# RemoteSensingTools/vSmartMOM.jl

Hardware: AMD Instinct MI355X
Metric: spectral-points/s (whole node) for rt_run, O2-A band (higher is better)
Workload: dtype f64; 1 GPU; C2: O2-A 759-770 nm, nStokes=3, Nquad=20 (N=60), 40 layers, 10000 spectral points/GPU, m=0..2, Rayleigh+synthetic O2 absorption, Lambertian 0.15; ranks=1, collective_backend=none (1 rank), N=60, layers=40, points_per_gpu=10000, fourier_moments=3

## Files before the change

include/vsmartmom_hip.h:

```cpp
#ifndef VSMARTMOM_HIP_H
#define VSMARTMOM_HIP_H

#include <stddef.h>
#include <stdint.h>

#ifdef __cplusplus
extern "C" {
#endif

typedef enum vsm_status {
  VSM_OK = 0,
  VSM_ERR_INVALID_ARG = 1,
  VSM_ERR_UNSUPPORTED = 2,
  VSM_ERR_HIP = 3,
  VSM_ERR_NO_DEVICE = 4
} vsm_status;

typedef enum vsm_iface {
  VSM_IFACE_00 = 0,
  VSM_IFACE_01 = 1,
  VSM_IFACE_10 = 2,
  VSM_IFACE_11 = 3
} vsm_iface;

// ... 334 lines not shown
                       size_t workspace_bytes, vsm_run** run);
int vsm_run_create_ex_f64(const vsm_quad_f64* q, int S, int nm, const int* m_h, const int* coupling_h, void* workspace,
                          size_t workspace_bytes, unsigned flags, vsm_run** run);
int vsm_run_create_ex_f32(const vsm_quad_f32* q, int S, int nm, const int* m_h, const int* coupling_h, void* workspace,
                          size_t workspace_bytes, unsigned flags, vsm_run** run);
int vsm_run_create_view_f64(const vsm_quad_f64* q, int S, int nm, const int* m_h, const int* coupling_h, void* workspace,
                            size_t workspace_bytes, unsigned flags, int nrows, const int* rows_h, vsm_run** run);
int vsm_run_create_view_f32(const vsm_quad_f32* q, int S, int nm, const int* m_h, const int* coupling_h, void* workspace,
                            size_t workspace_bytes, unsigned flags, int nrows, const int* rows_h, vsm_run** run);
int vsm_run_create_view_f64(const vsm_quad_f64* q, int S, int nm, const int* m_h, const int* coupling_h, void* workspace,
                            size_t workspace_bytes, unsigned flags, int nrows, const int* rows_h, vsm_run** run);
int vsm_run_create_view_f32(const vsm_quad_f32* q, int S, int nm, const int* m_h, const int* coupling_h, void* workspace,
                            size_t workspace_bytes, unsigned flags, int nrows, const int* rows_h, vsm_run** run);
int vsm_run_layer_f64(vsm_run* run, int ndoubl, const double* dtau, const double* varpi, const double* tau_sum,
                      const double* F0, int ncomp, const double* const* Zpp, const double* const* Zmp, long long z_stride,
                      const double* fcomp, int toa, const int* layer_coupling_h, void* stream);
int vsm_run_layer_f32(vsm_run* run, int ndoubl, const float* dtau, const float* varpi, const float* tau_sum,
                      const float* F0, int ncomp, const float* const* Zpp, const float* const* Zmp, long long z_stride,
                      const float* fcomp, int toa, const int* layer_coupling_h, void* stream);
int vsm_run_export_f64(vsm_run* run, const vsm_composite_f64* comps, void* stream);
int vsm_run_export_f32(vsm_run* run, const vsm_composite_f32* comps, void* stream);
int vsm_run_import_f64(vsm_run* run, const vsm_composite_f64* comps, void* stream);
int vsm_run_import_f32(vsm_run* run, const vsm_composite_f32* comps, void* stream);
int vsm_run_zw_tail(vsm_run* run);
int vsm_run_view_rows(vsm_run* run, int nrows, const int* rows_h);
int vsm_run_view_block(const vsm_run* run, int block, int* im, int* n, int* nv, int* local_rows);
int vsm_run_view_rows(vsm_run* run, int nrows, const int* rows_h);
int vsm_run_view_block(const vsm_run* run, int block, int* im, int* n, int* nv, int* local_rows);
int vsm_run_destroy(vsm_run* run);
int vsm_stokes_coupling_f64(int N, int n_stokes, int nblocks, const double* Zpp, const double* Zmp, int* mask_d, void* stream);
int vsm_stokes_coupling_f32(int N, int n_stokes, int nblocks, const float* Zpp, const float* Zmp, int* mask_d, void* stream);

typedef struct vsm_added_rs_f64 {
  double *ier_mp, *iet_pp, *ier_pm, *iet_mm;
  double *ieJ0_p, *ieJ0_m;
  int K;
  int reserved;
} vsm_added_rs_f64;
typedef struct vsm_added_rs_f32 {
  float *ier_mp, *iet_pp, *ier_pm, *iet_mm;
  float *ieJ0_p, *ieJ0_m;
  int K;
  int reserved;
} vsm_added_rs_f32;
typedef struct vsm_composite_rs_f64 {
  double *ieR_mp, *ieR_pm, *ieT_pp, *ieT_mm;
// ... 149 lines not shown
```

vsmartmom.jl_amd/_lib.py:

```python
from __future__ import annotations

import ctypes as C
import os

_HERE = os.path.dirname(os.path.abspath(__file__))
LIB_PATH = os.environ.get("VSM_LIB_PATH") or os.path.join(_HERE, "lib", "libvsmartmom_hip.so")


class VSMError(RuntimeError):
    pass


class vsm_quad_f64(C.Structure):
    _fields_ = [("mu", C.c_void_p), ("wt", C.c_void_p), ("N", C.c_int), ("n_stokes", C.c_int),
                ("i_mu0", C.c_int), ("mu0", C.c_double)]


class vsm_quad_f32(C.Structure):
    _fields_ = [("mu", C.c_void_p), ("wt", C.c_void_p), ("N", C.c_int), ("n_stokes", C.c_int),
                ("i_mu0", C.c_int), ("mu0", C.c_float)]


class vsm_added(C.Structure):
    _fields_ = [("r_mp", C.c_void_p), ("t_pp", C.c_void_p), ("r_pm", C.c_void_p), ("t_mm", C.c_void_p),
# ... 101 lines not shown
    "vsm_lambertian_surface_lin_{T}": (_I, [_P, _I, _I, "{R}", _I, _P, _P, _I, _P, _P, _P, _P]),
    "vsm_postprocess_vza_lin_{T}": (_I, [_I, _I, _I, _I, _I, _P, _P, _P, _P, _P, _P, _P]),
    "vsm_doubling_inelastic_work_elems": (_SZ, [_I, _I, _I]),
    "vsm_interaction_inelastic_work_elems": (_SZ, [_I, _I, _I]),
    "vsm_elemental_inelastic_rrs_{T}": (_I, [_P, _I, _I, _I, _P, _P, _P, _P, _P, _P]),
    "vsm_doubling_inelastic_rrs_{T}": (_I, [_I, _I, _I, _I, _P, _P, _P, _P, _P, _P]),
    "vsm_interaction_inelastic_rrs_{T}": (_I, [_I, _I, _I, _P, _P, _P, _P, _P, _P, _P]),
    "vsm_copy_added_to_composite_ie_{T}": (_I, [_I, _I, _P, _P, _P]),
    "vsm_postprocess_vza_ie_{T}": (_I, [_I, _I, _I, _I, _I, _P, _P, _P, _P, _P, _P, _P]),
    "vsm_ss_column_{T}": (_I, [_P, _I, _I, _I, _P, _P, _P, _P, _P, _P, _P, _P, _P, _P, _I, _P, _P, _P, _P, _P, _P, _P]),
    "vsm_ss_column_lin_{T}": (_I, [_P, _I, _I, _I, _I, _I, _I, _I, _I, _P, _P, _P, _P, _P, _P, _P, _P, _P, _P, _I, _P, _P, _P, _P, _P, _P, _P,
                                   _P, _P, _I, _P, _P, _P, _P, _P]),
    "vsm_ss_column_rrs_{T}": (_I, [_P, _I, _I, _I, _I, _P, _P, _P, _P, _P, _P, _P, _P, _I, _I, _P, _P, _P, _P, _P]),
    "vsm_run_supported": (_I, [_I, _I, _I]),
    "vsm_run_workspace_bytes": (_SZ, [_I, _I, _I, _I, _P]),
    "vsm_run_supported_f32": (_I, [_I, _I, _I]),
    "vsm_run_workspace_bytes_f32": (_SZ, [_I, _I, _I, _I, _P]),
    "vsm_run_create_{T}": (_I, [_P, _I, _I, _P, _P, _P, _SZ, _P]),
    "vsm_run_create_ex_{T}": (_I, [_P, _I, _I, _P, _P, _P, _SZ, C.c_uint, _P]),
    "vsm_run_create_view_{T}": (_I, [_P, _I, _I, _P, _P, _P, _SZ, C.c_uint, _I, _P, _P]),
    "vsm_run_layer_{T}": (_I, [_P, _I, _P, _P, _P, _P, _I, _P, _P, _LL, _P, _I, _P, _P]),
    "vsm_run_export_{T}": (_I, [_P, _P, _P]),
    "vsm_run_import_{T}": (_I, [_P, _P, _P]),
    "vsm_run_zw_tail": (_I, [_P]),
    "vsm_run_view_rows": (_I, [_P, _I, _P]),
    "vsm_run_view_block": (_I, [_P, _I, _P, _P, _P, _P]),
    "vsm_run_destroy": (_I, [_P]),
    "vsm_stokes_coupling_{T}": (_I, [_I, _I, _I, _P, _P, _P, _P]),
    "vsm_level_radiance_work_elems": (_SZ, [_I, _I]),
    "vsm_level_radiance_{T}": (_I, [_I, _I, _I, _I, _P, _P, _P, _P, _P, _LL, _P, _P, _P, _P, _P, _P, _P]),
    "vsm_level_radiance_oplevel_{T}": (_I, [_I, _I, _I, _I, _P, _P, _P, _P, _P, _LL, _P, _P, _P, _P, _P, _P, _P]),
    "vsm_level_radiance_src_{T}": (_I, [_I, _I, _I, _I, _P, _P, _P, _I, _P, _P, _LL, _P, _P, _P, _P, _P, _P, _P]),
    "vsm_level_radiance_ie_{T}": (_I, [_I, _I, _I, _I, _P, _I, _P, _P, _P, _P, _LL, _P, _P, _P, _P, _P, _P, _P, _P, _P, _P, _P]),
    "vsm_level_radiance_lin_{T}": (_I, [_I, _I, _I, _I, _I, _I, _P, _P, _P, _P, _LL, _P, _P, _P, _LL, _P, _P, _LL, _LL, _P, _P, _P, _P, _P,
                                        _P]),
    "vsm_test_lds_mm_{T}": (_I, [_I, _I, _P, _P, _P, _P]),
    "vsm_test_lds_inv_{T}": (_I, [_I, _I, _P, _P, _I, _P, _P]),
    "vsm_test_poison_lds": (_I, [_P]),
}


def exported_symbols():
    out = []
    for name in _SIGS:
        if "{T}" in name:
            out += [name.format(T="f64"), name.format(T="f32")]
# ... 89 lines not shown
```

vsmartmom.jl_amd/core_rt.py:

```python
from __future__ import annotations

import ctypes as C
import dataclasses
import math
import os
from dataclasses import dataclass
from typing import List, Optional

import numpy as np
import torch

from . import _lib
from . import host_model as H
from .architectures import GPU, CPU, architecture, array_type, devi, synchronize_if_gpu, to_host

IFACE = {"00": 0, "01": 1, "10": 2, "11": 3}
MOMENT_BATCH = 4
MOMENT_BATCH_MAX = 24
MOMENT_BATCHING = True
THERMAL_FUSION = True
NATIVE_RUN = True
NATIVE_SOURCES_ONLY = True
NATIVE_VIEW_ROWS = True
VIEW_ROWS_MAX = 16
NATIVE_ZW_TAIL = True
NATIVE_DROPIN = True
REFERENCE_ORDER = False


def _require_gpu(arch):
    if not isinstance(arch, GPU):
        raise _lib.VSMError("vsmartmom.jl_amd provides the MI355X path only; architecture %r has no compute path here "
                            "(no CPU fallback by design)" % (arch,))
    if not torch.cuda.is_available():
        raise _lib.VSMError("no MI355X visible to HIP (torch.cuda.is_available() is False)")
    if arch.device_index != torch.cuda.current_device():
        raise _lib.VSMError("architecture GPU(%d) is not the current HIP device (%d): one process per GPU -- call "
                            "torch.cuda.set_device(%d) first" % (arch.device_index, torch.cuda.current_device(),
                                                                 arch.device_index))


def _torch_dtype(FT):
    return torch.float64 if np.dtype(FT) == np.float64 else torch.float32


def _stream_ptr():
    return C.c_void_p(torch.cuda.current_stream().cuda_stream)
# ... 76 lines not shown
class AddedLayer:

    def __init__(self, FT, arch, N, nSpec, shared=False, d_symmetric=0):
        dev, dt = devi(arch), _torch_dtype(FT)
        sm = 1 if shared else nSpec
        z = lambda: torch.zeros((sm, N, N), dtype=dt, device=dev)
        self.r_mp, self.t_pp = z(), z()
        self.d_symmetric = int(d_symmetric)
        self.r_pm, self.t_mm = (None, None) if self.d_symmetric else (z(), z())
        self.j0_p = torch.zeros((nSpec, N), dtype=dt, device=dev)
        self.j0_m = torch.zeros((nSpec, N), dtype=dt, device=dev)
        self.N, self.nSpec, self.shared, self.dtype = N, nSpec, shared, dt

    def cstruct(self):
        return _lib.vsm_added(self.r_mp.data_ptr(), self.t_pp.data_ptr(),
                              0 if self.r_pm is None else self.r_pm.data_ptr(),
                              0 if self.t_mm is None else self.t_mm.data_ptr(),
                              self.j0_p.data_ptr(), self.j0_m.data_ptr(), 0 if self.shared else self.N * self.N,
                              self.d_symmetric, 0)


def _composite_field(name):
    def fget(self):
        return self.materialize()._arr[name]

    def fset(self, value):
        self.materialize()._arr[name] = value
    return property(fget, fset)


class CompositeLayer:

    def __init__(self, FT, arch, N, nSpec):
        dev, dt = devi(arch), _torch_dtype(FT)
        z = lambda: torch.zeros((nSpec, N, N), dtype=dt, device=dev)
        self._native = None
        self._sources_only = False
        self._view_rows = None
        self._native_ws = None
        self._arr = dict(R_mp=z(), R_pm=z(), T_pp=z(), T_mm=z(), J0_p=torch.zeros((nSpec, N), dtype=dt, device=dev),
                         J0_m=torch.zeros((nSpec, N), dtype=dt, device=dev))
        self.N, self.nSpec, self.dtype = N, nSpec, dt

    R_mp, R_pm, T_pp = _composite_field("R_mp"), _composite_field("R_pm"), _composite_field("T_pp")
    T_mm, J0_p, J0_m = _composite_field("T_mm"), _composite_field("J0_p"), _composite_field("J0_m")

    def materialize(self):
        slot = self._native
        if slot is None:
            return self
        self._native = None
        try:
            cc = (_lib.vsm_composite * 1)(self._cstruct_raw())
            _lib.call("vsm_run_export", self.dtype, slot.run, cc, _stream_ptr())
        finally:
            _lib.lib().vsm_run_destroy(slot.run)
        return self

    def drop_native(self):
        slot, self._native = self._native, None
        if slot is not None:
            _lib.lib().vsm_run_destroy(slot.run)

    def _cstruct_raw(self):
        a = self._arr
        return _lib.vsm_composite(a["R_mp"].data_ptr(), a["R_pm"].data_ptr(), a["T_pp"].data_ptr(), a["T_mm"].data_ptr(),
                                  a["J0_p"].data_ptr(), a["J0_m"].data_ptr())

    def cstruct(self):
        self.materialize()
        return self._cstruct_raw()

    def __del__(self):
        try:
            self.drop_native()
        except Exception:
            pass


def make_added_layer(FT, arch, dims, nSpec, shared=False, d_symmetric=0) -> AddedLayer:
    _require_gpu(arch)
    return AddedLayer(FT, arch, dims[0], nSpec, shared, d_symmetric)


def make_composite_layer(FT, arch, dims, nSpec) -> CompositeLayer:
    _require_gpu(arch)
    return CompositeLayer(FT, arch, dims[0], nSpec)


@dataclass
class DeviceLayerOptics:
    tau: torch.Tensor
    varpi: torch.Tensor
    Zpp: torch.Tensor
# ... 77 lines not shown

_work_cache = {}


def layer_forward_multi_(tau_sum, dtau, F0, props_list, ms, ndoubl: int, dq: DeviceQuad, toa: bool, comps, added: AddedLayer):
    nm = len(ms)
    p0 = props_list[0]
    q, a = dq.cstruct(), added.cstruct()
    dtype = comps[0].dtype
    carr = (type(comps[0].cstruct()) * nm)(*[c.cstruct() for c in comps])
    marr = (C.c_int * nm)(*[int(m) for m in ms])
    zpp = (C.c_void_p * nm)(*[p.Zpp.data_ptr() for p in props_list])
    zmp = (C.c_void_p * nm)(*[p.Zmp.data_ptr() for p in props_list])
    ncomp = 0 if p0.fcomp is None else int(p0.fcomp.shape[1])
    _lib.call("vsm_layer_forward_multi", dtype, C.byref(q), comps[0].nSpec, nm, marr, ndoubl, _ptr(dtau), _ptr(p0.varpi),
              _ptr(tau_sum), _ptr(F0), ncomp, zpp, zmp, 0 if ncomp else p0.z_stride, _ptr(p0.fcomp), None, 1 if toa else 0,
              carr, C.byref(a), _stream_ptr())


def run_layer_native_(run, nm: int, ndoubl: int, dtau, varpi, tau_sum, F0, ncomp: int, zpp, zmp, z_stride: int, fcomp, toa: bool,
                      layer_coupling=None, dtype=torch.float64):
    _lib.call("vsm_run_layer", dtype, run, ndoubl, _ptr(dtau), _ptr(varpi), _ptr(tau_sum), _ptr(F0), ncomp, zpp, zmp, z_stride,
              _ptr(fcomp), 1 if toa else 0, layer_coupling, _stream_ptr())


def interaction_(scattering_interface: str, comp: CompositeLayer, added: AddedLayer, oplevel: bool = False,
                 work: Optional[torch.Tensor] = None):
    a, c = added.cstruct(), comp.cstruct()
    N, S = comp.N, comp.nSpec
    fused = (scattering_interface == "11" and not oplevel
             and N <= _lib.lib().vsm_fused_max_n(8 if comp.dtype == torch.float64 else 4))
    if not fused and work is None:
        key = (N, S, comp.dtype, str(comp.R_mp.device))
        work = _work_cache.get(key)
        if work is None:
            _work_cache.clear()
            work = _lib.poison(torch.empty(int(_lib.lib().vsm_interaction_work_elems(N, S)), dtype=comp.dtype, device=comp.R_mp.device))
            _work_cache[key] = work
    name = "vsm_interaction_oplevel" if oplevel else "vsm_interaction"
    _lib.call(name, comp.dtype, IFACE[scattering_interface], N, S, C.byref(c), C.byref(a), _ptr(work), _stream_ptr())


_phi_cache = {}


def brdf_azimuth_quadrature(arch, FT):
# ... 39 lines not shown
        _lib.call("vsm_lambertian_surface_spectral", added_surface.dtype, C.byref(q), added_surface.nSpec, m, _ptr(rho),
                  _ptr(tau_sum), C.byref(a), _stream_ptr())
        return
    if not added_surface.shared:
        raise _lib.VSMError("surface AddedLayer must be allocated with shared=True")
    if isinstance(surface, H.LambertianSurfaceScalar):
        surface = surface.albedo
    if isinstance(surface, (int, float)):
        alb = C.c_double(surface) if added_surface.dtype == torch.float64 else C.c_float(surface)
        _lib.call("vsm_lambertian_surface", added_surface.dtype, C.byref(q), added_surface.nSpec, m, alb, _ptr(tau_sum),
                  C.byref(a), _stream_ptr())
        return
    if isinstance(surface, BRDF_SURFACES):
        if rho is None:
            rho, _ = reflectance(surface, dq, m, arch, FT)
        _lib.call("vsm_brdf_surface", added_surface.dtype, C.byref(q), added_surface.nSpec, m, _ptr(rho), _ptr(tau_sum),
                  C.byref(a), _stream_ptr())
        return
    raise _lib.VSMError("surface %r is not built in this backend (LambertianSurfaceScalar / Legendre / Spline, CoxMunkSurface, "
                        "rpvSurfaceScalar, RossLiSurfaceScalar)"
                        % (surface,))


def apply_ss_correction_(R_SFI: torch.Tensor, surf: H.CoxMunkSurface, pol, vza, vaz, mu0, tau_total: torch.Tensor, m_max: int,
                         arch, FT):
    nV, S = len(vza), int(R_SFI.shape[0])
    ctype = C.c_double if R_SFI.dtype == torch.float64 else C.c_float
    mu_v = (ctype * nV)(*[float(FT(H.cosd(v))) for v in vza])
    dph = (ctype * nV)(*[float(FT(math.radians(float(a)))) for a in vaz])
    coef = torch.empty((pol.n, nV), dtype=R_SFI.dtype, device=R_SFI.device)
    phi, w = brdf_azimuth_quadrature(arch, FT)
    cs = _coxmunk_cstruct(surf, R_SFI.dtype)
    _lib.call("vsm_coxmunk_ss_correction", R_SFI.dtype, C.byref(cs), pol.n, S, nV, mu_v, dph, ctype(float(mu0)), int(m_max),
              int(phi.numel()), _ptr(phi), _ptr(w), _ptr(tau_total), _ptr(coef), _ptr(R_SFI), _stream_ptr())
    return coef


def postprocessing_vza_(pol: H.PolarizationType, comp: CompositeLayer, vza, vaz, qp: H.QuadPoints, m: int, weight: float,
                        R_SFI: torch.Tensor, T_SFI: torch.Tensor):
    n, nV = pol.n, len(vza)
    row0 = (C.c_int * nV)()
    ctype = C.c_double if comp.dtype == torch.float64 else C.c_float
    w = (ctype * (nV * n))()
    for v in range(nV):
        imu = int(np.argmin(np.abs(qp.qp_mu - qp.qp_mu.dtype.type(H.cosd(vza[v])))))
        row0[v] = imu * n
# ... 1 lines not shown
        ws = [c, c, s, s][:n]
        for k in range(n):
            w[v + nV * k] = weight * ws[k]
    _lib.call("vsm_postprocess_vza", comp.dtype, comp.N, n, comp.nSpec, nV, row0, w, _ptr(comp.J0_m), _ptr(comp.J0_p),
              _ptr(R_SFI), _ptr(T_SFI), _stream_ptr())


def _vza_rows_weights(pol, vza, vaz, qp, m, weight, dtype):
    n, nV = pol.n, len(vza)
    row0 = (C.c_int * nV)()
    ctype = C.c_double if dtype == torch.float64 else C.c_float
    w = (ctype * (nV * n))()
    for v in range(nV):
        imu = int(np.argmin(np.abs(qp.qp_mu - qp.qp_mu.dtype.type(H.cosd(vza[v])))))
        row0[v] = imu * n
        c, s = H.cosd(m * vaz[v]), H.sind(m * vaz[v])
        for k in range(n):
            w[v + nV * k] = weight * [c, c, s, s][k]
    return row0, w


def interaction_hdrf_(pol, comp: CompositeLayer, added_surface: AddedLayer, m: int, dq: DeviceQuad, vza, vaz, qp, weight: float,
                      hdr_J: torch.Tensor, hdr: torch.Tensor, bhr_uw: torch.Tensor, bhr_dw: torch.Tensor):
    q, c, a = dq.cstruct(), comp.cstruct(), added_surface.cstruct()
    _lib.call("vsm_interaction_hdrf", comp.dtype, C.byref(q), comp.nSpec, m, C.byref(c), C.byref(a), _ptr(hdr_J), _ptr(bhr_uw),
              _ptr(bhr_dw), _stream_ptr())
    row0, w = _vza_rows_weights(pol, vza, vaz, qp, m, weight, comp.dtype)
    _lib.call("vsm_postprocess_vza_hdrf", comp.dtype, comp.N, pol.n, comp.nSpec, len(vza), row0, w, _ptr(hdr_J), _ptr(hdr),
              _stream_ptr())


def init_layer(props: DeviceLayerOptics, qp: H.QuadPoints, FT, numerics: H.RTNumericalParameters, arch):
    dtau_h, nd = H.get_dtau_ndoubl(props.tau_h, props.varpi_h, qp, FT, numerics)
    return array_type(arch)(dtau_h), nd


@dataclass
class NativeSlot:
    run: C.c_void_p
    m: int
    coupling: int
    grp_of: List[int]


def stokes_groups(n_stokes: int, coupling: int) -> List[int]:
    adj = [[a == b or coupling < 0 or bool((coupling >> (4 * a + b)) & 1) or bool((coupling >> (4 * b + a)) & 1)
            for b in range(n_stokes)] for a in range(n_stokes)]
# ... 378 lines not shown
        if self.layers_only:
            raise _lib.VSMError("Scene(layers_only=True) holds no composite layer: it feeds rt_run_ss only")
        self.R_SFI.zero_()
        self.T_SFI.zero_()
        self.hdr.zero_()
        if self.S == 0:
            return self.R_SFI, self.T_SFI
        self.added.j0_p.zero_()
        eps2 = 2 * np.finfo(FT).eps
        has_noscat = any(ly["props"].max_tau_varpi <= eps2 for ly in self.moments[0]["layers"])
        sequential = trace is not None or not MOMENT_BATCHING or has_noscat or REFERENCE_ORDER
        want = max(MOMENT_BATCH, min(MOMENT_BATCH_MAX, 4096 // max(self.S, 1)))
        nb = 1 if sequential else min(want, len(self.moments))
        while len(self._composites) < nb:
            self._composites.append(make_composite_layer(FT, self.arch, (self.N, self.N), self.S))
        native = self._native_moments() if trace is None and not has_noscat and not REFERENCE_ORDER else set()
        walk_src = streams is None and trace is None and not has_noscat
        if getattr(self, "_view_rows", None) is None:
            self._view_rows = view_rows_of(pol, model.vza, self.qp)
        view_rows = self._view_rows if streams is None else None
        for c in self._composites:
            c._sources_only = walk_src and REFERENCE_ORDER
            c._view_rows = view_rows if c._sources_only else None
        for g0 in range(0, len(self.moments), nb):
            group = self.moments[g0:g0 + nb]
            comps = self._composites[:len(group)]
            nat = [k for k in range(len(group)) if (g0 + k) in native]
            if nat:
                self._run_layers_native([group[k] for k in nat], [comps[k] for k in nat], sources_only=streams is None,
                                        view_rows=view_rows)
            rest = [k for k in range(len(group)) if (g0 + k) not in native]
            group_l, comps_l = [group[k] for k in rest], [comps[k] for k in rest]
            for iz in range(self.Nz if rest else 0):
                ly0 = group_l[0]["layers"][iz]
                if len(group_l) > 1 and ly0["props"].max_tau_varpi > eps2 and (iz == 0 or ly0["iface"] == "11"):
                    layer_forward_multi_(ly0["tau_sum"], ly0["dtau"], self.F0, [mom["layers"][iz]["props"] for mom in group_l],
                                         [mom["m"] for mom in group_l], ly0["nd"], self.dq, iz == 0, comps_l, self.added)
                    continue
                for mom, comp in zip(group_l, comps_l):
                    ly = mom["layers"][iz]
                    rt_kernel_(pol, self.added, comp, ly["props"], ly["iface"], ly["tau_sum"], mom["m"], self.dq,
                               self.arch, iz + 1, self.F0, FT, model.numerics, dtau=ly["dtau"], ndoubl=ly["nd"], trace=trace,
                               work=self.work, keep_added=has_noscat)
            for mom, comp in zip(group, comps):
                m = mom["m"]
                weight = FT(0.5 / math.pi) if m == 0 else FT(1.0 / math.pi)
                create_surface_layer_(model.surface, self.added_surface, m, self.dq, mom["tau_sum_surface"], rho=mom["rho"])
                interaction_(mom["iface_surface"], comp, self.added_surface, work=self.work)
                if self.compute_hdrf:
                    interaction_hdrf_(pol, comp, self.added_surface, m, self.dq, model.vza, model.vaz, self.qp, float(weight),
                                      self.hdr_J, self.hdr, self.bhr_uw, self.bhr_dw)
                postprocessing_vza_(pol, comp, model.vza, model.vaz, self.qp, m, float(weight), self.R_SFI, self.T_SFI)
                thermal_pass = self.thermal_B is not None and (m == 0 or (m == 1 and self._thermal_carry))
                if thermal_pass:
                    self._thermal_slot(mom, float(weight))
                if streams is not None:
                    Jm, Jp = comp.J0_m.clone(), comp.J0_p.clone()
                    if thermal_pass:
                        Jm += self._th_comp.J0_m
                        Jp += self._th_comp.J0_p
                    streams.append(dict(m=m, weight=float(weight), R_mp=comp.R_mp.clone(), T_pp=comp.T_pp.clone(), J0_m=Jm, J0_p=Jp))
        for c in self._composites:
            c._sources_only = False
            c._view_rows = None
        if isinstance(model.surface, H.CoxMunkSurface) and self.ss_correction:
            apply_ss_correction_(self.R_SFI, model.surface, pol, model.vza, model.vaz, self.qp.mu0,
                                 self.moments[-1]["tau_sum_surface"], model.m_max, self.arch, FT)
        return self.R_SFI, self.T_SFI

    def _native_moments(self):
        if not NATIVE_RUN or getattr(self, "coupling", None) is None or not self.moments:
            return set()
        eps2 = 2 * np.finfo(self.FT).eps
        for iz, ly in enumerate(self.moments[0]["layers"]):
            p = ly["props"]
            if p.max_tau_varpi <= eps2 or (iz > 0 and ly["iface"] != "11") or (p.fcomp is not None and p.fcomp.shape[1] > 4):
                return set()
        return {i for i, mom in enumerate(self.moments) if run_supported(self.dt, self.N, self.pol.n, int(self.coupling[mom["m"]]))}

    def _run_layers_native(self, group, comps, sources_only: bool = True, export_at=None, view_rows=None):
        L = _lib.lib()
        nm, N, S, ns = len(group), self.N, self.S, self.pol.n
        marr = (C.c_int * nm)(*[int(mom["m"]) for mom in group])
        carr = (C.c_int * nm)(*[int(self.coupling[mom["m"]]) for mom in group])
        nbytes = run_workspace_bytes(self.dt, N, ns, S, nm, carr)
        ws = getattr(self, "_native_ws", None)
        if ws is None or ws.numel() * 8 < nbytes:
            ws = self._native_ws = _lib.poison(torch.empty(max(nbytes // 8, 2), dtype=torch.float64, device=self.dev))
        q = self.dq.cstruct()
        run = C.c_void_p()
        run_create_(self.dt, q, S, nm, marr, carr, ws, nbytes, sources_only, view_rows, run)
        try:
            if NATIVE_ZW_TAIL and not torch.cuda.is_current_stream_capturing():
                _lib.check(L.vsm_run_zw_tail(run))
            for iz in range(self.Nz):
                ly0 = group[0]["layers"][iz]
                props = [mom["layers"][iz]["props"] for mom in group]
                p0 = props[0]
                zpp = (C.c_void_p * nm)(*[p.Zpp.data_ptr() for p in props])
                zmp = (C.c_void_p * nm)(*[p.Zmp.data_ptr() for p in props])
                ncomp = 0 if p0.fcomp is None else int(p0.fcomp.shape[1])
                lc = (C.c_int * nm)(*[self._layer_coupling(mom["m"], iz) for mom in group])
                run_layer_native_(run, nm, int(ly0["nd"]), ly0["dtau"], p0.varpi, ly0["tau_sum"], self.F0, ncomp, zpp, zmp,
                                  0 if ncomp else p0.z_stride, p0.fcomp, iz == 0, lc, self.dt)
                if export_at and (iz + 1) in export_at:
                    cc = (type(comps[0].cstruct()) * nm)(*[c.cstruct() for c in comps])
                    _lib.call("vsm_run_export", self.dt, run, cc, _stream_ptr())
                    export_at[iz + 1](comps)
            cc = (type(comps[0].cstruct()) * nm)(*[c.cstruct() for c in comps])
            _lib.call("vsm_run_export", self.dt, run, cc, _stream_ptr())
        finally:
            L.vsm_run_destroy(run)

    def _thermal_slot(self, mom, weight):
        self._thermal_begin(mom)
        comp = self._th_comp
        self._thermal_walk(mom, comp, 0, self.Nz)
        surf = self._thermal_surface(mom)
        interaction_(mom["iface_surface"], comp, surf, oplevel=True, work=self.work)
        postprocessing_vza_(self.pol, comp, self.model.vza, self.model.vaz, self.qp, mom["m"], weight, self.R_SFI, self.T_SFI)

    def _thermal_begin(self, mom):
        N, S, FT = self.N, self.S, self.FT
        if getattr(self, "_th_added", None) is None:
            self._th_added = make_added_layer(FT, self.arch, (N, N), S, d_symmetric=0)
            self._th_surf = make_added_layer(FT, self.arch, (N, N), S, shared=not self.spectral_surface)
            self._th_comp = make_composite_layer(FT, self.arch, (N, N), S)
            self._th_F0 = torch.zeros_like(self.F0)
            self._th_ones = torch.ones(max(S, 1), dtype=self.dt, device=self.dev)
        if mom["m"] == 0:
            eps2 = 2 * np.finfo(FT).eps
            scat = [ly["props"].max_tau_varpi > eps2 for ly in mom["layers"]]
            self._th_added.j0_p.zero_()
# ... 138 lines not shown
```

vsmartmom.jl_amd/core_rt_ms.py:

```python
from __future__ import annotations

import ctypes as C
import math
from dataclasses import dataclass
from typing import List

import numpy as np
import torch

from . import _lib
from . import core_rt as CR
from . import host_model as H
from .architectures import synchronize_if_gpu, to_host

LEVEL_FUSED_MAX_N = 128
LEVEL_OPLEVEL = False


class _CompositeAsAdded:

    def __init__(self, comp: CR.CompositeLayer):
        self.comp = comp

    def cstruct(self):
# ... 249 lines not shown
    scene.T_SFI.zero_()
    weights = []
    if S == 0:
        return out, full, [float(fourier_weight(FT, m)) for m in range(model.m_max + 1)]
    scene.added.j0_p.zero_()
    sequential = not CR.MOMENT_BATCHING or CR.REFERENCE_ORDER
    want = max(CR.MOMENT_BATCH, min(CR.MOMENT_BATCH_MAX, 4096 // max(S, 1)))
    nb = 1 if sequential else min(want, len(scene.moments))
    thermal = scene.thermal_B is not None
    if tops_at and dev.type == "cuda":
        elt = torch.finfo(dt).bits // 8
        per_moment = len(tops_at) * (N * N + N) * S * elt + (4 * N * N + 2 * N) * S * elt
        if thermal:
            per_moment += len(tops_at) * N * S * elt
        free = torch.cuda.mem_get_info(dev)[0]
        nb = max(1, min(nb, int(0.5 * free // per_moment)))
    while len(scene._composites) < nb:
        scene._composites.append(CR.make_composite_layer(FT, scene.arch, (N, N), S))
    segs = [CR.make_composite_layer(FT, scene.arch, (N, N), S) for _ in range(2 if plan.interior else 0)]
    th_of = {id(seg): CR.make_composite_layer(FT, scene.arch, (N, N), S) for seg in segs} if thermal else {}
    native = scene._native_moments() if not CR.REFERENCE_ORDER else set()
    for c in scene._composites:
        c._sources_only = CR.REFERENCE_ORDER
    try:
        for g0 in range(0, len(scene.moments), nb):
            group = scene.moments[g0:g0 + nb]
            comps = scene._composites[:len(group)]
            tops = [dict() for _ in group]
            nat = [k for k in range(len(group)) if (g0 + k) in native]
            if nat:
                def keep(l):
                    def cb(cs):
                        for k, c in zip(nat, cs):
                            tops[k][l] = (c._arr["R_pm"].clone(), c._arr["J0_p"].clone())
                    return cb
                scene._run_layers_native([group[k] for k in nat], [comps[k] for k in nat], sources_only=True,
                                         export_at={l: keep(l) for l in tops_at})
            rest = [k for k in range(len(group)) if (g0 + k) not in native]
            group_l, comps_l = [group[k] for k in rest], [comps[k] for k in rest]
            for iz in range(Nz if rest else 0):
                ly0 = group_l[0]["layers"][iz]
                if len(group_l) > 1 and (iz == 0 or ly0["iface"] == "11"):
                    CR.layer_forward_multi_(ly0["tau_sum"], ly0["dtau"], scene.F0, [mom["layers"][iz]["props"] for mom in group_l],
                                            [mom["m"] for mom in group_l], ly0["nd"], scene.dq, iz == 0, comps_l, scene.added)
                else:
                    for mom, comp in zip(group_l, comps_l):
# ... 86 lines not shown
```

vsmartmom.jl_amd/csrc/vsm_native.hip:

```cpp
#include <stdlib.h>

#include <vector>

#include "vsm_native_dev.h"
#include "vsm_native_run.h"

#ifndef VSM_NATIVE_PARK_RT
#define VSM_NATIVE_PARK_RT 3
#endif

namespace vsm {

struct nlayer_comps {
  double* c[NSUB_MAX];
};

namespace {

template <int RT, int KS, int KZ = KS>
__device__ __forceinline__ void ned_body(nsmem<RT, (4 * KS + 2 > 16 * RT)>& sm, npos<RT>& p, int n, int gsz, unsigned uvmask, int ndoubl,
                                         const double* __restrict__ img, nstrip<RT>& r_s, nstrip<RT>& t_s, int* status) {
  using G = ngeo<RT>;
  constexpr unsigned dP = 0, dQ = G::AF * 8;
  double* jp = sm.vec[0];
// ... 1224 lines not shown
      const T* cn = gm.base[gi] + (long long)s * (4 * af + 2 * np);
      const int js = (j / ns) * gm.gsz[gi] + gm.pos_in[aj];
      const int ix = nat_idx_rt(cn, rt, is, js);
#pragma unroll
      for (int k = 0; k < 4; ++k)
        if (!(view && k == NC_TMM)) v[k] = cn[k * af + ix];
      if (view && at >= 0) v[NC_TMM] = cn[NC_TMM * af + at * np + js];
    }
    if (src) v[NC_RMP] = v[NC_TPP] = (T)__builtin_nan("");
    if (view && at < 0) v[NC_TMM] = (T)__builtin_nan("");
#pragma unroll
    for (int k = 0; k < 4; ++k) out[k][e] = v[k];
  }
  if (tid < N) {
    const int ai = tid % ns, gi = gm.grp_of[ai];
    const int rt = gm.rt[gi], np = 16 * rt, af = np * np;
    const T* cn = gm.base[gi] + (long long)s * (4 * af + 2 * np);
    const int is = (tid / ns) * gm.gsz[gi] + gm.pos_in[ai];
    c.J0_p[(long long)s * N + tid] = cn[4 * af + is];
    c.J0_m[(long long)s * N + tid] = (view && vw.find(gi, is) < 0) ? (T)__builtin_nan("") : cn[4 * af + np + is];
  }
}
template <typename T>
__global__ __launch_bounds__(256) void k_native_import(int N, int ns, int view, ngroup_map<T> gm, nview vw, composite<T> c) {
  const int s = blockIdx.x, tid = threadIdx.x;
  const long long NN = (long long)N * N;
  const T* in[4] = {c.R_mp + s * NN, c.R_pm + s * NN, c.T_pp + s * NN, c.T_mm + s * NN};
  for (int g = 0; g < gm.ngroups; ++g) {
    const int rt = gm.rt[g], np = 16 * rt, af = np * np, n = gm.n[g], gsz = gm.gsz[g];
    T* cn = gm.base[g] + (long long)s * (4 * af + 2 * np);
    int comp_of[4] = {0, 0, 0, 0};
    for (int a = 0; a < ns; ++a)
      if (gm.grp_of[a] == g) comp_of[gm.pos_in[a]] = a;
    for (int e = tid; e < af; e += 256) {
      const int is = e % np, js = e / np;
      T v[4] = {0, 0, 0, 0};
      if (is < n && js < n) {
        const int i = (is / gsz) * ns + comp_of[is % gsz], j = (js / gsz) * ns + comp_of[js % gsz];
#pragma unroll
        for (int k = 0; k < 4; ++k) v[k] = in[k][i + (long long)N * j];
      }
      const int ix = nat_idx_rt(cn, rt, is, js);
#pragma unroll
      for (int k = 0; k < 4; ++k)
        if (!(view && k == NC_TMM)) cn[k * af + ix] = v[k];
    }
// ... 506 lines not shown
    npre_args<T> pa;
    T* lc[NSUB_MAX];
    for (int k = 0; k < NSUB_MAX; ++k) {
      const nat_sub& sb = run->subs[act[k < nsub ? k : 0]];
      pa.s[k].m = sb.m;
      pa.s[k].gsz = sb.gsz;
      for (int a = 0; a < 4; ++a) pa.s[k].g[a] = sb.g[a];
      VSM_REQUIRE(Zpp[sb.im] && Zmp[sb.im], "vsm_run_layer: null Z of moment %d", sb.im);
      pa.s[k].z = zsrc<T>{Zpp[sb.im], Zmp[sb.im], ncomp ? 0 : z_stride, ncomp, fcomp};
      lc[k] = ws + sb.comp_off;
    }
    T* pre_cl = pre + off;
    off += pre_stride_rt(h.rt) * (size_t)run->S * nsub;
    native_launch_pre(h.rt, ncomp > 0, q, run->S, nsub, h.n, ndoubl, dtau, varpi, tau_sum, F0, pa, pre_cl, st);
    VSM_LAUNCH_CHECK("k_elemental_native");
    const nview vw = view ? view_of(run, act) : nview{};
    const int rc = native_launch_layer(h, run->S, nsub, ndoubl, toa, src, pre_cl, lc, status, view ? &vw : nullptr, st);
    if (rc) return rc;
  }
  return VSM_OK;
}

template <typename T, typename CS, bool IMPORT>
static int run_convert(vsm_run* run, const CS* comps, void* stream) {
  VSM_REQUIRE(run && comps, "vsm_run_export / import: null argument");
  VSM_REQUIRE(run->elem_size == (int)sizeof(T), "vsm_run_export / import: the run was created for %d-byte arrays", run->elem_size);
  if (IMPORT) ++run->imports;
  if (run->S == 0) return VSM_OK;
  if (IMPORT) {
    run->pure_diag.assign(run->subs.size(), 0);
    run->flags &= ~(unsigned)VSM_RUN_ZW_TAIL;
    for (nat_sub& sb : run->subs) sb.kz = sb.ks;
  }
  for (int im = 0; im < run->nm; ++im) {
    const CS& c = comps[im];
    VSM_REQUIRE(c.R_mp && c.R_pm && c.T_pp && c.T_mm && c.J0_p && c.J0_m, "vsm_run_export / import: null composite array (moment %d)", im);
    const composite<T> cc{c.R_mp, c.R_pm, c.T_pp, c.T_mm, c.J0_p, c.J0_m};
    const ngroup_map<T> gm = group_map<T>(run, im);
    const int view = (run->flags & VSM_RUN_VIEW_ROWS) ? 1 : 0;
    const nview vw = view ? view_of_moment(run, im) : nview{};
    if (IMPORT)
      hipLaunchKernelGGL((k_native_import<T>), dim3(run->S), dim3(256), 0, as_stream(stream), run->N, run->ns, view, gm, vw, cc);
    else
      hipLaunchKernelGGL((k_native_export<T>), dim3(run->S), dim3(256), 0, as_stream(stream), run->N, run->ns,
                         (run->flags & VSM_RUN_SOURCES_ONLY) ? 1 : 0, view, gm, vw, cc);
    VSM_LAUNCH_CHECK("k_native_export / import");
  }
  return VSM_OK;
}

template <typename T>
static int stokes_coupling(int N, int n_stokes, int nblocks, const T* Zpp, const T* Zmp, int* mask_d, void* stream) {
  VSM_REQUIRE(N > 0 && n_stokes >= 1 && n_stokes <= 4 && N % n_stokes == 0 && nblocks >= 1 && nblocks <= 65535 && Zpp && Zmp &&
                  mask_d, "vsm_stokes_coupling: bad argument");
  hipStream_t st = as_stream(stream);
  VSM_HIP(hipMemsetAsync(mask_d, 0, sizeof(int) * nblocks, st));
  const long long tot = (long long)N * N;
  const int blocks = (int)((tot + 255) / 256 < 16 ? (tot + 255) / 256 : 16);
  hipLaunchKernelGGL((k_stokes_coupling<T>), dim3(blocks, nblocks), dim3(256), 0, st, N, n_stokes, Zpp, Zmp, mask_d);
  VSM_LAUNCH_CHECK("k_stokes_coupling");
  return VSM_OK;
}

}
}

using namespace vsm;

extern "C" {
// ... 86 lines not shown
                      int ncomp, const double* const* Zpp, const double* const* Zmp, long long z_stride, const double* fcomp,
                      int toa, const int* layer_coupling, void* stream) {
  return run_layer<double>(run, ndoubl, dtau, varpi, tau_sum, F0, ncomp, Zpp, Zmp, z_stride, fcomp, toa, layer_coupling, stream);
}
int vsm_run_layer_f32(vsm_run* run, int ndoubl, const float* dtau, const float* varpi, const float* tau_sum, const float* F0,
                      int ncomp, const float* const* Zpp, const float* const* Zmp, long long z_stride, const float* fcomp,
                      int toa, const int* layer_coupling, void* stream) {
  return run_layer<float>(run, ndoubl, dtau, varpi, tau_sum, F0, ncomp, Zpp, Zmp, z_stride, fcomp, toa, layer_coupling, stream);
}

int vsm_run_export_f64(vsm_run* run, const vsm_composite_f64* comps, void* stream) {
  return run_convert<double, vsm_composite_f64, false>(run, comps, stream);
}
int vsm_run_export_f32(vsm_run* run, const vsm_composite_f32* comps, void* stream) {
  return run_convert<float, vsm_composite_f32, false>(run, comps, stream);
}
int vsm_run_import_f64(vsm_run* run, const vsm_composite_f64* comps, void* stream) {
  return run_convert<double, vsm_composite_f64, true>(run, comps, stream);
}
int vsm_run_import_f32(vsm_run* run, const vsm_composite_f32* comps, void* stream) {
  return run_convert<float, vsm_composite_f32, true>(run, comps, stream);
}

int vsm_stokes_coupling_f64(int N, int n_stokes, int nblocks, const double* Zpp, const double* Zmp, int* mask_d, void* stream) {
  return stokes_coupling<double>(N, n_stokes, nblocks, Zpp, Zmp, mask_d, stream);
}
int vsm_stokes_coupling_f32(int N, int n_stokes, int nblocks, const float* Zpp, const float* Zmp, int* mask_d, void* stream) {
  return stokes_coupling<float>(N, n_stokes, nblocks, Zpp, Zmp, mask_d, stream);
}

}

#endif
```

Before: 26440 spectral-points/s.

## Skip surface interaction and matrix export for zero-transmission Lambertian moments

For Fourier moments m>=1 with a Lambertian surface, the surface layer is identically zero, so the surface interaction and the export of the composite R/T matrices are skipped. A new sources-only export kernel copies just J0+ and J0-, and the full matrix export runs only for moments that still need it. The skipped composites are flagged stale so any later read of their matrices raises an error. This avoids N×N matrix copies and a surface interaction per spectral point for m=1,2, at the cost of extra state-tracking complexity.

Result: no change. 26660 spectral-points/s (median of 6 runs) (+0.8%).

```diff
diff --git a/include/vsmartmom_hip.h b/include/vsmartmom_hip.h
--- a/include/vsmartmom_hip.h
+++ b/include/vsmartmom_hip.h
@@ -380,6 +380,10 @@
 int vsm_run_export_f32(vsm_run* run, const vsm_composite_f32* comps, void* stream);
 int vsm_run_import_f64(vsm_run* run, const vsm_composite_f64* comps, void* stream);
 int vsm_run_import_f32(vsm_run* run, const vsm_composite_f32* comps, void* stream);
+int vsm_run_export_sources_f64(vsm_run* run, const vsm_composite_f64* comps, void* stream);
+int vsm_run_export_sources_f32(vsm_run* run, const vsm_composite_f32* comps, void* stream);
+int vsm_run_export_moment_f64(vsm_run* run, int im, const vsm_composite_f64* comp, void* stream);
+int vsm_run_export_moment_f32(vsm_run* run, int im, const vsm_composite_f32* comp, void* stream);
 int vsm_run_zw_tail(vsm_run* run);
 int vsm_run_view_rows(vsm_run* run, int nrows, const int* rows_h);
 int vsm_run_view_block(const vsm_run* run, int block, int* im, int* n, int* nv, int* local_rows);
diff --git a/vsmartmom.jl_amd/_lib.py b/vsmartmom.jl_amd/_lib.py
--- a/vsmartmom.jl_amd/_lib.py
+++ b/vsmartmom.jl_amd/_lib.py
@@ -147,6 +147,8 @@
     "vsm_run_layer_{T}": (_I, [_P, _I, _P, _P, _P, _P, _I, _P, _P, _LL, _P, _I, _P, _P]),
     "vsm_run_export_{T}": (_I, [_P, _P, _P]),
     "vsm_run_import_{T}": (_I, [_P, _P, _P]),
+    "vsm_run_export_sources_{T}": (_I, [_P, _P, _P]),
+    "vsm_run_export_moment_{T}": (_I, [_P, _I, _P, _P]),
     "vsm_run_zw_tail": (_I, [_P]),
     "vsm_run_view_rows": (_I, [_P, _I, _P]),
     "vsm_run_view_block": (_I, [_P, _I, _P, _P, _P, _P]),
diff --git a/vsmartmom.jl_amd/core_rt.py b/vsmartmom.jl_amd/core_rt.py
--- a/vsmartmom.jl_amd/core_rt.py
+++ b/vsmartmom.jl_amd/core_rt.py
@@ -23,6 +23,7 @@
 NATIVE_SOURCES_ONLY = True
 NATIVE_VIEW_ROWS = True
 VIEW_ROWS_MAX = 16
+NATIVE_SURFACE = True
 NATIVE_ZW_TAIL = True
 NATIVE_DROPIN = True
 REFERENCE_ORDER = False
@@ -145,11 +146,16 @@
 
 def _composite_field(name):
     def fget(self):
+        if name in _COMPOSITE_MATRICES:
+            self._require_matrices(name)
         return self.materialize()._arr[name]
 
     def fset(self, value):
         self.materialize()._arr[name] = value
     return property(fget, fset)
+
+
+_COMPOSITE_MATRICES = ("R_mp", "R_pm", "T_pp", "T_mm")
 
 
 class CompositeLayer:
@@ -161,6 +167,7 @@
         self._sources_only = False
         self._view_rows = None
         self._native_ws = None
+        self._stale_matrices = False
         self._arr = dict(R_mp=z(), R_pm=z(), T_pp=z(), T_mm=z(), J0_p=torch.zeros((nSpec, N), dtype=dt, device=dev),
                          J0_m=torch.zeros((nSpec, N), dtype=dt, device=dev))
         self.N, self.nSpec, self.dtype = N, nSpec, dt
@@ -190,9 +197,23 @@
         return _lib.vsm_composite(a["R_mp"].data_ptr(), a["R_pm"].data_ptr(), a["T_pp"].data_ptr(), a["T_mm"].data_ptr(),
                                   a["J0_p"].data_ptr(), a["J0_m"].data_ptr())
 
-    def cstruct(self):
+    def cstruct(self, sources: bool = False):
+        if not sources:
+            self._require_matrices("cstruct()")
         self.materialize()
         return self._cstruct_raw()
+
+    def mark_stale(self):
+        self._stale_matrices = True
+
+    def reuse(self):
+        self._stale_matrices = False
+
+    def _require_matrices(self, what):
+        if self._stale_matrices:
+            raise _lib.VSMError("CompositeLayer.%s: the run that filled this composite exported J0+- alone (core_rt.NATIVE_SURFACE: "
+                                "the moment's surface layer is exactly zero, nothing reads the matrices); its R-+, R+-, T++, T-- "
+                                "are stale.  Run with `streams=`, or with NATIVE_SURFACE = False, to get them" % what)
 
     def __del__(self):
         try:
@@ -316,6 +337,14 @@
                       layer_coupling=None, dtype=torch.float64):
     _lib.call("vsm_run_layer", dtype, run, ndoubl, _ptr(dtau), _ptr(varpi), _ptr(tau_sum), _ptr(F0), ncomp, zpp, zmp, z_stride,
               _ptr(fcomp), 1 if toa else 0, layer_coupling, _stream_ptr())
+
+
+def run_export_sources_(run, cc, dtype=torch.float64):
+    _lib.call("vsm_run_export_sources", dtype, run, cc, _stream_ptr())
+
+
+def run_export_moment_(run, im: int, c, dtype=torch.float64):
+    _lib.call("vsm_run_export_moment", dtype, run, int(im), C.byref(c), _stream_ptr())
 
 
 def interaction_(scattering_interface: str, comp: CompositeLayer, added: AddedLayer, oplevel: bool = False,
@@ -401,6 +430,16 @@
                         % (surface,))
 
 
+def surface_zero_transmission(surface, m: int):
+    if m < 1:
+        return None
+    if isinstance(surface, (H.LambertianSurfaceLegendre, H.LambertianSurfaceSpline)):
+        return 0.0
+    if isinstance(surface, H.LambertianSurfaceScalar) or (isinstance(surface, (int, float)) and not isinstance(surface, bool)):
+        return 1.0
+    return None
+
+
 def apply_ss_correction_(R_SFI: torch.Tensor, surf: H.CoxMunkSurface, pol, vza, vaz, mu0, tau_total: torch.Tensor, m_max: int,
                          arch, FT):
     nV, S = len(vza), int(R_SFI.shape[0])
@@ -448,7 +487,7 @@
 
 def interaction_hdrf_(pol, comp: CompositeLayer, added_surface: AddedLayer, m: int, dq: DeviceQuad, vza, vaz, qp, weight: float,
                       hdr_J: torch.Tensor, hdr: torch.Tensor, bhr_uw: torch.Tensor, bhr_dw: torch.Tensor):
-    q, c, a = dq.cstruct(), comp.cstruct(), added_surface.cstruct()
+    q, c, a = dq.cstruct(), comp.cstruct(sources=True), added_surface.cstruct()
     _lib.call("vsm_interaction_hdrf", comp.dtype, C.byref(q), comp.nSpec, m, C.byref(c), C.byref(a), _ptr(hdr_J), _ptr(bhr_uw),
               _ptr(bhr_dw), _stream_ptr())
     row0, w = _vza_rows_weights(pol, vza, vaz, qp, m, weight, comp.dtype)
@@ -873,13 +912,24 @@
         for c in self._composites:
             c._sources_only = walk_src and REFERENCE_ORDER
             c._view_rows = view_rows if c._sources_only else None
+        surf_native = (NATIVE_SURFACE and NATIVE_SOURCES_ONLY and walk_src and not REFERENCE_ORDER and self.dt == torch.float64
+                       and self.thermal_B is None)
         for g0 in range(0, len(self.moments), nb):
             group = self.moments[g0:g0 + nb]
             comps = self._composites[:len(group)]
+            for c in comps:
+                c.reuse()
             nat = [k for k in range(len(group)) if (g0 + k) in native]
+            zero_t = {}
+            if nat and surf_native:
+                for k in nat:
+                    zt = surface_zero_transmission(model.surface, group[k]["m"]) if group[k]["iface_surface"] == "11" else None
+                    if zt is not None:
+                        zero_t[k] = zt
             if nat:
                 self._run_layers_native([group[k] for k in nat], [comps[k] for k in nat], sources_only=streams is None,
-                                        view_rows=view_rows)
+                                        view_rows=view_rows,
+                                        sources_moments={i for i, k in enumerate(nat) if k in zero_t} if zero_t else None)
             rest = [k for k in range(len(group)) if (g0 + k) not in native]
             group_l, comps_l = [group[k] for k in rest], [comps[k] for k in rest]
             for iz in range(self.Nz if rest else 0):
@@ -893,11 +943,14 @@
                     rt_kernel_(pol, self.added, comp, ly["props"], ly["iface"], ly["tau_sum"], mom["m"], self.dq,
                                self.arch, iz + 1, self.F0, FT, model.numerics, dtau=ly["dtau"], ndoubl=ly["nd"], trace=trace,
                                work=self.work, keep_added=has_noscat)
-            for mom, comp in zip(group, comps):
+            for k, (mom, comp) in enumerate(zip(group, comps)):
                 m = mom["m"]
                 weight = FT(0.5 / math.pi) if m == 0 else FT(1.0 / math.pi)
                 create_surface_layer_(model.surface, self.added_surface, m, self.dq, mom["tau_sum_surface"], rho=mom["rho"])
-                interaction_(mom["iface_surface"], comp, self.added_surface, work=self.work)
+                if k not in zero_t:
+                    interaction_(mom["iface_surface"], comp, self.added_surface, work=self.work)
+                elif zero_t[k] == 0.0:
+                    comp._arr["J0_p"].zero_()
                 if self.compute_hdrf:
                     interaction_hdrf_(pol, comp, self.added_surface, m, self.dq, model.vza, model.vaz, self.qp, float(weight),
                                       self.hdr_J, self.hdr, self.bhr_uw, self.bhr_dw)
@@ -929,8 +982,10 @@
                 return set()
         return {i for i, mom in enumerate(self.moments) if run_supported(self.dt, self.N, self.pol.n, int(self.coupling[mom["m"]]))}
 
-    def _run_layers_native(self, group, comps, sources_only: bool = True, export_at=None, view_rows=None):
+    def _run_layers_native(self, group, comps, sources_only: bool = True, export_at=None, view_rows=None, sources_moments=None):
         L = _lib.lib()
+        for c in comps:
+            c.reuse()
         nm, N, S, ns = len(group), self.N, self.S, self.pol.n
         marr = (C.c_int * nm)(*[int(mom["m"]) for mom in group])
         carr = (C.c_int * nm)(*[int(self.coupling[mom["m"]]) for mom in group])
@@ -959,7 +1014,17 @@
                     _lib.call("vsm_run_export", self.dt, run, cc, _stream_ptr())
                     export_at[iz + 1](comps)
             cc = (type(comps[0].cstruct()) * nm)(*[c.cstruct() for c in comps])
-            _lib.call("vsm_run_export", self.dt, run, cc, _stream_ptr())
+            if sources_moments:
+                if not (sources_only and NATIVE_SOURCES_ONLY and self.dt == torch.float64):
+                    raise _lib.VSMError("_run_layers_native: sources_moments needs a sources-only FP64 run")
+                run_export_sources_(run, cc, self.dt)
+                for k in range(nm):
+                    if k in sources_moments:
+                        comps[k].mark_stale()
+                    else:
+                        run_export_moment_(run, k, cc[k], self.dt)
+            else:
+                _lib.call("vsm_run_export", self.dt, run, cc, _stream_ptr())
         finally:
             L.vsm_run_destroy(run)
 
diff --git a/vsmartmom.jl_amd/core_rt_ms.py b/vsmartmom.jl_amd/core_rt_ms.py
--- a/vsmartmom.jl_amd/core_rt_ms.py
+++ b/vsmartmom.jl_amd/core_rt_ms.py
@@ -295,6 +295,7 @@
     native = scene._native_moments() if not CR.REFERENCE_ORDER else set()
     for c in scene._composites:
         c._sources_only = CR.REFERENCE_ORDER
+        c.reuse()
     try:
         for g0 in range(0, len(scene.moments), nb):
             group = scene.moments[g0:g0 + nb]
diff --git a/vsmartmom.jl_amd/csrc/vsm_native.hip b/vsmartmom.jl_amd/csrc/vsm_native.hip
--- a/vsmartmom.jl_amd/csrc/vsm_native.hip
+++ b/vsmartmom.jl_amd/csrc/vsm_native.hip
@@ -1270,6 +1270,20 @@
   }
 }
 template <typename T>
+__global__ __launch_bounds__(256) void k_native_export_sources(int N, int ns, int S, int view, ngroup_map<T> gm, nview vw,
+                                                               T* __restrict__ J0_p, T* __restrict__ J0_m) {
+  const long long e = blockIdx.x * 256ll + threadIdx.x;
+  if (e >= (long long)N * S) return;
+  const int i = (int)(e % N);
+  const long long s = e / N;
+  const int ai = i % ns, gi = gm.grp_of[ai];
+  const int rt = gm.rt[gi], np = 16 * rt, af = np * np;
+  const T* cn = gm.base[gi] + s * (4 * af + 2 * np);
+  const int is = (i / ns) * gm.gsz[gi] + gm.pos_in[ai];
+  J0_p[e] = cn[4 * af + is];
+  J0_m[e] = (view && vw.find(gi, is) < 0) ? (T)__builtin_nan("") : cn[4 * af + np + is];
+}
+template <typename T>
 __global__ __launch_bounds__(256) void k_native_import(int N, int ns, int view, ngroup_map<T> gm, nview vw, composite<T> c) {
   const int s = blockIdx.x, tid = threadIdx.x;
   const long long NN = (long long)N * N;
@@ -1822,6 +1836,22 @@
 }
 
 template <typename T, typename CS, bool IMPORT>
+static int convert_moment(vsm_run* run, int im, const CS& c, void* stream) {
+  VSM_REQUIRE(c.R_mp && c.R_pm && c.T_pp && c.T_mm && c.J0_p && c.J0_m, "vsm_run_export / import: null composite array (moment %d)", im);
+  const composite<T> cc{c.R_mp, c.R_pm, c.T_pp, c.T_mm, c.J0_p, c.J0_m};
+  const ngroup_map<T> gm = group_map<T>(run, im);
+  const int view = (run->flags & VSM_RUN_VIEW_ROWS) ? 1 : 0;
+  const nview vw = view ? view_of_moment(run, im) : nview{};
+  if (IMPORT)
+    hipLaunchKernelGGL((k_native_import<T>), dim3(run->S), dim3(256), 0, as_stream(stream), run->N, run->ns, view, gm, vw, cc);
+  else
+    hipLaunchKernelGGL((k_native_export<T>), dim3(run->S), dim3(256), 0, as_stream(stream), run->N, run->ns,
+                       (run->flags & VSM_RUN_SOURCES_ONLY) ? 1 : 0, view, gm, vw, cc);
+  VSM_LAUNCH_CHECK("k_native_export / import");
+  return VSM_OK;
+}
+
+template <typename T, typename CS, bool IMPORT>
 static int run_convert(vsm_run* run, const CS* comps, void* stream) {
   VSM_REQUIRE(run && comps, "vsm_run_export / import: null argument");
   VSM_REQUIRE(run->elem_size == (int)sizeof(T), "vsm_run_export / import: the run was created for %d-byte arrays", run->elem_size);
@@ -1833,18 +1863,36 @@
     for (nat_sub& sb : run->subs) sb.kz = sb.ks;
   }
   for (int im = 0; im < run->nm; ++im) {
-    const CS& c = comps[im];
-    VSM_REQUIRE(c.R_mp && c.R_pm && c.T_pp && c.T_mm && c.J0_p && c.J0_m, "vsm_run_export / import: null composite array (moment %d)", im);
-    const composite<T> cc{c.R_mp, c.R_pm, c.T_pp, c.T_mm, c.J0_p, c.J0_m};
+    const int rc = convert_moment<T, CS, IMPORT>(run, im, comps[im], stream);
+    if (rc) return rc;
+  }
+  return VSM_OK;
+}
+
+template <typename T, typename CS>
+static int run_export_moment(vsm_run* run, int im, const CS* comp, void* stream) {
+  VSM_REQUIRE(run && comp, "vsm_run_export_moment: null argument");
+  VSM_REQUIRE(run->elem_size == (int)sizeof(T), "vsm_run_export_moment: the run was created for %d-byte arrays", run->elem_size);
+  VSM_REQUIRE(im >= 0 && im < run->nm, "vsm_run_export_moment: moment index %d outside 0 .. %d", im, run->nm - 1);
+  if (run->S == 0) return VSM_OK;
+  return convert_moment<T, CS, false>(run, im, *comp, stream);
+}
+
+template <typename T, typename CS>
+static int run_export_sources(vsm_run* run, const CS* comps, void* stream) {
+  VSM_REQUIRE(run && comps, "vsm_run_export_sources: null argument");
+  VSM_REQUIRE(run->elem_size == (int)sizeof(T), "vsm_run_export_sources: the run was created for %d-byte arrays", run->elem_size);
+  for (int im = 0; im < run->nm; ++im)
+    VSM_REQUIRE(comps[im].J0_p && comps[im].J0_m, "vsm_run_export_sources: null J0+ / J0- (moment %d)", im);
+  if (run->S == 0) return VSM_OK;
+  const int view = (run->flags & VSM_RUN_VIEW_ROWS) ? 1 : 0;
+  const long long tot = (long long)run->N * run->S;
+  for (int im = 0; im < run->nm; ++im) {
     const ngroup_map<T> gm = group_map<T>(run, im);
-    const int view = (run->flags & VSM_RUN_VIEW_ROWS) ? 1 : 0;
     const nview vw = view ? view_of_moment(run, im) : nview{};
-    if (IMPORT)
-      hipLaunchKernelGGL((k_native_import<T>), dim3(run->S), dim3(256), 0, as_stream(stream), run->N, run->ns, view, gm, vw, cc);
-    else
-      hipLaunchKernelGGL((k_native_export<T>), dim3(run->S), dim3(256), 0, as_stream(stream), run->N, run->ns,
-                         (run->flags & VSM_RUN_SOURCES_ONLY) ? 1 : 0, view, gm, vw, cc);
-    VSM_LAUNCH_CHECK("k_native_export / import");
+    hipLaunchKernelGGL((k_native_export_sources<T>), dim3((unsigned)((tot + 255) / 256)), dim3(256), 0, as_stream(stream), run->N,
+                       run->ns, run->S, view, gm, vw, comps[im].J0_p, comps[im].J0_m);
+    VSM_LAUNCH_CHECK("k_native_export_sources");
   }
   return VSM_OK;
 }
@@ -1977,6 +2025,19 @@
   return run_convert<float, vsm_composite_f32, true>(run, comps, stream);
 }
 
+int vsm_run_export_sources_f64(vsm_run* run, const vsm_composite_f64* comps, void* stream) {
+  return run_export_sources<double, vsm_composite_f64>(run, comps, stream);
+}
+int vsm_run_export_sources_f32(vsm_run* run, const vsm_composite_f32* comps, void* stream) {
+  return run_export_sources<float, vsm_composite_f32>(run, comps, stream);
+}
+int vsm_run_export_moment_f64(vsm_run* run, int im, const vsm_composite_f64* comp, void* stream) {
+  return run_export_moment<double, vsm_composite_f64>(run, im, comp, stream);
+}
+int vsm_run_export_moment_f32(vsm_run* run, int im, const vsm_composite_f32* comp, void* stream) {
+  return run_export_moment<float, vsm_composite_f32>(run, im, comp, stream);
+}
+
 int vsm_stokes_coupling_f64(int N, int n_stokes, int nblocks, const double* Zpp, const double* Zmp, int* mask_d, void* stream) {
   return stokes_coupling<double>(N, n_stokes, nblocks, Zpp, Zmp, mask_d, stream);
 }
```
